# TakiRyo/object-triggered-3D-SLAM

Hardware: AMD Instinct MI355X
Metric: RGB-D frames/sec (640×480, 5mm voxel TSDF) at 1/2/4/8 GPU; Mpoints/s filtered (higher is better)
Workload: dtype f32 tsdf/weight + f64 colour; 1 GPU; configs[1]: 256-frame 640x480 RGB-D TSDF integration, 5 mm voxel, sdf_trunc 0.04, one object scan per GPU (synthetic box-on-floor ring scan), colour precision 64 (Open3D's float64 TSDFVoxel::color_, exact division: bit-exact colours); color_precision=64, width=640, height=480, volume_units=5896, parallelism=objects1

## Files before the change

### object-triggered-3d-slam_amd/_lib.py

```python
from __future__ import annotations

import ctypes as C
import os
import threading

_HERE = os.path.dirname(os.path.abspath(__file__))
LIB_PATH = os.path.join(_HERE, "libotslam_hip.so")
HEADER_PATH = os.path.join(os.path.dirname(_HERE), "include", "otslam.h")

OT_OK = 0
OT_ERR_INVALID_ARGUMENT = 1
OT_ERR_UNSUPPORTED_FORMAT = 2
OT_ERR_CAPACITY = 3
OT_ERR_HIP = 4

OT_COLOR_NONE = 0
OT_COLOR_RGB8 = 1


class ot_intrinsics(C.Structure):
    _fields_ = [("width", C.c_int32), ("height", C.c_int32), ("fx", C.c_double), ("fy", C.c_double),
                ("cx", C.c_double), ("cy", C.c_double)]


# ... 56 lines not shown
    "ot_tsdf_import_units": [_p, _i64, _p, _p, _p, _p, _p],
    "ot_tsdf_import_units_color64": [_p, _i64, _p, _p, _p, _p, _p],
    "ot_tsdf_set_shard": [_p, _i32, _i32],
    "ot_tsdf_set_shard_block": [_p, _i32],
    "ot_tsdf_set_shard_sector": [_p, _i32, _i32, _d, _d],
    "ot_tsdf_batch_stats": [_p, _pi64, _pi64, _pi64],
    "ot_tsdf_border_destinations": [_p, _i64, _p, _p, _p],
    "ot_tsdf_mesh_serial": [_p, _pi64],
    "ot_tsdf_mesh_vertex_normals": [_p, _i64, _p, _i64, _p, _i64, _p, _p],
    "ot_tsdf_export_border": [_p, _i64, _p, _p, _p, _p, _pi64, _p],
    "ot_tsdf_import_border": [_p, _i64, _p, _p, _p, _p, _p],
    "ot_tsdf_fetch_mesh_keys": [_p, _p, _p, _p],
    "ot_tsdf_extract_triangle_mesh": [_p, _pi64, _pi64, _p],
    "ot_tsdf_fetch_triangle_mesh": [_p, _p, _p, _p, _p],
    "ot_tsdf_extract_triangle_mesh_count": [_p, _pi64, _pi64, _p],
    "ot_tsdf_emit_triangle_mesh": [_p, _p, _p, _p, _p],
    "ot_tsdf_extract_triangle_mesh_into": [_p, _p, _p, _p, _i64, _i64, _pi64, _pi64, _p],
    "ot_tsdf_extract_sample_min_z": [_p, _p, _p, _p, _i64, _i64, _p, _p, _i64, C.c_uint64, _d, _p, _p, _pi64, _pi64,
                                     _pi64, _p],
    "ot_tsdf_extract_point_cloud_count": [_p, _pi64, _p],
    "ot_tsdf_emit_point_cloud": [_p, _p, _p, _p, _p],
    "ot_tsdf_extract_voxel_point_cloud_count": [_p, _pi64, _p],
    "ot_tsdf_emit_voxel_point_cloud": [_p, _p, _p, _p],
    "ot_mesh_compute_vertex_normals": [_p, _i64, _p, _i64, _p, _p],
    "ot_mesh_sample_points_uniformly": [_p, _p, _p, _i64, _p, _i64, _i64, C.c_uint64, _p, _p, _p, _p],
    "ot_mesh_sample_points_uniformly_batch": [_p, _i32, _i64, C.c_uint64, _p],
    "ot_mesh_sample_points_min_z": [_p, _i32, _i64, C.c_uint64, _d, _pi64, _p],
    "ot_mesh_sample_points_min_z_async": [_p, _i32, _i64, C.c_uint64, _d, _p],
    "ot_mesh_sample_points_min_z_wait": [_i32, _pi64],
    "ot_mesh_sample_points_uniformly_after": [_p, _i32, _i64, C.c_uint64, _p, _p],
    "ot_mesh_get_surface_area": [_p, _i64, _p, _i64, C.POINTER(C.c_double), _p],
    "ot_mesh_cluster_connected_triangles": [_p, _i64, _p, _i64, _p, _p, _p, _pi64, _p],
    "ot_mesh_flag_degenerate_triangles": [_p, _i64, _i64, _p, _p],
    "ot_mesh_flag_duplicated_triangles": [_p, _i64, _i64, _p, _p],
    "ot_mesh_remove_triangles_by_mask": [_p, _i64, _p, _p, _pi64, _p],
    "ot_mesh_remove_unreferenced_vertices": [_i64, _p, _i64, _p, _pi64, _p],
    "ot_occupancy_to_points": [_p, _i32, _i32, _i32, _d, _d, _d, _p, _pi64, _p],
    "ot_grid_smart_paste": [_p, _p, _i32, _i32, _i32, _i32, _i32, _i32, _i32, _i32, _pi64, _p],
    "ot_voxel_key_diff": [_p, _i64, _p, _i64, _d, _p, _p, _pi64, _p, _pi64, _p],
    "ot_voxel_key_diff_multi": [_p, _p, _p, _p, _i32, _d, _p, _p, _pi64, _p, _pi64, _p],
    "ot_scan_diff": [_p, _p, _i32, _i32, C.c_float, C.c_float, C.c_float, C.c_float, C.c_float, _d, _i32, _p, _d,
                     _p, _p, _p, _p, _p],
    "ot_virtual_scan": [_p, _i32, _i32, C.c_float, C.c_float, C.c_float, _i32, _i32, C.c_float, C.c_float,
                        C.c_float, _p, _p, _p],
    "ot_change_grid_create": [_d, _d, _d, C.POINTER(_p)],
    "ot_change_grid_destroy": [_p],
    "ot_change_grid_update": [_p, _p, _p, _i64, _d],
    "ot_change_grid_publish": [_p, _p, _i64, _pi64],
    "ot_scan_cluster": [_p, _i32, _i32, C.c_float, C.c_float, C.c_float, _p, _p, _p, _p, _p, _p, _p, _p, _p, _p, _p,
                        _p],
    "ot_object_map_filter": [_p, _p, _i32, _p, _i32, C.c_float, C.c_float, C.c_float, _p, _d, _p, _p, _p, _p],
    "ot_cluster_observations": [_p, _i32, _p, _i32, _p, _p, _p, _p, _p],
    "ot_rgbd_filter_create": [_pint, _i32, _d, _d, _d, _i32, _d, C.POINTER(_p)],
    "ot_rgbd_filter_destroy": [_p],
    "ot_rgbd_filter_run": [_p, _i32, _p, _p, _p, _p],
    "ot_rgbd_filter_sizes": [_p, _pi64, _pi64, _pi64, _p, _p, _p],
    "ot_rgbd_filter_outputs": [_p, C.POINTER(_p), C.POINTER(_p), C.POINTER(_p), C.POINTER(_p), C.POINTER(_p),
                               C.POINTER(_p)],
    "ot_rgbd_filter_copy": [_p, _i32, _p, _p, _p, _p, _p, _p, _p],
}
_RESTYPES = {"ot_last_error": C.c_char_p, "ot_version": C.c_char_p, "ot_abi_version": C.c_int32,
             "otx_alloc_count": C.c_longlong}

_lib = None
_lock = threading.Lock()


class OTError(RuntimeError):
    """Raised for any non-OK status; message mirrors Open3D's utility::LogError text."""


TEST_SIGNATURES = {
    "otx_serial_chain_f64": [_p, _i64, _i32, _p, _pi64, _p],
    "otx_chain_walk_trace": [_p, _i64, _i32, _p, _p, _i32, _p],
    "otx_tsdf_stats": [_p, _p],
    "otx_unit_sort_radix": [_i32],
    "otx_sor_netfill": [_i32],
    "otx_integrate_fine": [_i32],
    "otx_integrate_workgroup": [_i32],
    "otx_touch_stage_blocks": [_i32],
    "otx_touch_frames": [_i32],
    "otx_split_frontend": [_i32],
    "otx_slice_pretest": [_i32],
    "otx_defer_integrate": [_i32],
    "otx_integrate_depth": [_i32],
    "otx_mc_emit_fork": [_i32],
    "otx_normals_at": [_i32],
    "otx_sampler_hi_stream": [_i32],
    "otx_sort_pairs_u64_u32": [_p, _p, _p, _p, _i64, _i32, _p],
    "otx_sort_segments_u32_u32": [_p, _p, _p, _p, _p, _i32, _i32, _p],
    "otx_alloc_count": [],
    "otx_registration_last_d2": [_p, _i64, _p],
}


def use_variant(path: str) -> None:
    global LIB_PATH
    path = os.path.abspath(path)
    if os.path.dirname(path) != os.path.join(_HERE, "variants"):
        raise RuntimeError(f"variant libraries live in {os.path.join(_HERE, 'variants')}: {path}")
    if _lib is not None:
        raise RuntimeError("use_variant() after the library was loaded")
    LIB_PATH = path


def load():
    global _lib
    if _lib is not None:
        return _lib
    with _lock:
        if _lib is not None:
            return _lib
        if not os.path.exists(LIB_PATH):
            raise RuntimeError(f"HIP extension missing: {LIB_PATH} (run __graft_entry__.build())")
        lib = C.CDLL(LIB_PATH)
        lib.ot_version.argtypes, lib.ot_version.restype = [], C.c_char_p
        built, src = library_source_hash(lib), source_hash()
        if built != src:
            raise RuntimeError(f"stale HIP library {LIB_PATH}: built from sources {built or '(no hash)'}, "
                               f"sources here are {src} (run __graft_entry__.build())")
        missing = []
        for name, argtypes in {**SIGNATURES, **TEST_SIGNATURES}.items():
            try:
                f = getattr(lib, name)
            except AttributeError:
                missing.append(name)
                continue
            f.argtypes = argtypes
            f.restype = _RESTYPES.get(name, C.c_int32)
        lib._ot_missing = set(missing)
        _lib = lib
    return _lib


def call(name, *args):
    lib = load()
    if name in lib._ot_missing:
        raise RuntimeError(f"{LIB_PATH} does not export {name} (stale build?)")
    st = getattr(lib, name)(*args)
    if st != OT_OK:
        msg = lib.ot_last_error().decode(errors="replace")
        raise OTError(msg or f"{name} failed with status {st}")
    return st


def alloc_count() -> int:
    return int(load().otx_alloc_count())


def intrinsics_struct(intr) -> ot_intrinsics:
    return ot_intrinsics(int(intr.width), int(intr.height), float(intr.fx), float(intr.fy), float(intr.cx),
                         float(intr.cy))


def source_hash() -> str:
    from . import _srchash

    return _srchash.compute()


def library_source_hash(lib) -> str:
    ver = lib.ot_version().decode(errors="replace")
    return ver.rsplit(" src=", 1)[1].strip() if " src=" in ver else ""
```

### object-triggered-3d-slam_amd/csrc/tsdf.h

```cpp
#pragma once

#include <vector>

#include "common.h"

namespace ot {

constexpr int UNIT_RES = 16;
constexpr int UNIT_VOX = UNIT_RES * UNIT_RES * UNIT_RES;
constexpr int UNIT_FIELDS = 5;
constexpr int UNIT_FLOATS = UNIT_FIELDS * UNIT_VOX;
constexpr int UNIT_FLOATS_C64 = 8 * UNIT_VOX;

constexpr int C_UNUSED0 = 0;
constexpr int C_UNITS = 1;
constexpr int C_OVERFLOW = 2;
constexpr int C_HASHERR = 3;
constexpr int C_BATCH_PAIRS = 4;
constexpr int C_ORDER_HEAVY = 6;
constexpr int C_ORDER_LIGHT = 7;
constexpr int C_KMAX = 8;
constexpr int C_KNEG = 11;
constexpr int C_UNITS_DONE = 14;
constexpr int N_COUNTERS = 16;
// ... 83 lines not shown
    }
    return -1;
}

__device__ inline int hash_find(const TsdfDev& d, unsigned long long key) {
    unsigned slot = (unsigned)mix64(key) & (unsigned)d.hash_mask;
    for (int probe = 0; probe <= d.hash_mask; ++probe) {
        const unsigned long long k = d.hkeys[slot];
        if (k == key) return (int)slot;
        if (k == KEY_EMPTY) return -1;
        slot = (slot + 1) & (unsigned)d.hash_mask;
    }
    return -1;
}

__host__ __device__ inline float* unit_base(const TsdfDev& d, int id) { return d.vox + (size_t)id * d.unit_floats; }
template <typename CT>
__device__ inline CT* color_base(const TsdfDev& d, int id) {
    return reinterpret_cast<CT*>(unit_base(d, id) + 2 * UNIT_VOX);
}

constexpr int BORDER_VOX = 721;
__host__ __device__ inline void border_voxel(int b, int& x, int& y, int& z) {
    if (b < 256) {
        x = 0, y = b >> 4, z = b & 15;
        return;
    }
    const int c = b - 256, r = c % 31;
    x = 1 + c / 31;
    if (r < 16) y = 0, z = r;
    else y = r - 15, z = 0;
}

constexpr int MAX_BATCH = 64;
constexpr int OT_MAIL_WORDS = 64;
constexpr int MAIL_SEQ_MC = OT_MAIL_WORDS - 2;
constexpr int MAIL_SEQ_UNITS = 2 * OT_MAIL_WORDS - 1;

struct BatchFrame {
    const uint16_t* depth16;
    const float* depthf;
    const uint8_t* color;
    uint2* dc;
    uint64_t pad;
    double pose[12];
    float E[12];
    float es[3];
    float scale;
    double trunc;
};

struct IntegrateParams {
    const float* depth;
    const uint8_t* color;
    const float* mult;
    int W, H;
    float fx, fy, cx, cy;
    float E[12];
    float es0, es1, es2;
    float vl, half, trunc, trunc_inv, safe_w, safe_h;
    float inv_fx, inv_fy;
    float proj_eps;
    int rcp_hi;
    double unit_len;
    const unsigned* tmax;
    int tmax_tiles;
    int tmax_words;
};

struct BatchTouchParams {
    int W, stride, ws, hs;
    double fx, fy, cx, cy;
    double trunc, unit_len;
    double inv_unit;
    int slot_cap;
    int64_t npx;
    int pc;
    int tiles;
    int stage_blocks;
    int tf;
    int sample_stage;
    unsigned* tmax;
    int H;
};

struct StageMaskParams {
    int W, H, tiles_x, tiles_y, wpr;
    float fx, fy, cx, cy, vl, half;
    double unit_len;
    int nframes;
};

struct UnitWork {
    int id;
    int kx, ky, kz;
    unsigned long long mask;
    unsigned long long pad;
};

enum class BatchMode { Direct, Overlap, Deferred };
struct BatchPlan {
    BatchMode mode = BatchMode::Direct;
    bool split = false;
    bool pretest = false;
    int set = 0;
    int* wcount = nullptr;
    int* wcopy = nullptr;
};

struct BatchCtx {
    BatchPlan plan;
    BatchTouchParams tp;
    IntegrateParams ip0;
    StageMaskParams sq{};
    unsigned* smask = nullptr;
    int n, pc, variant;
};

struct PendingFrame {
    const uint16_t* depth;
    const float* depthf;
    const uint8_t* color;
    ot_intrinsics intr;
    double extrinsic[16];
    double depth_scale, depth_trunc;
};

struct MeshBuffers {
    void* ws = nullptr;
    size_t ws_bytes = 0;
    int64_t ws_units = 0;
    int64_t serial = 0;
    bool valid = false;
    bool internal = false;
    bool emitted = false;
    double* v = nullptr;
    double* c = nullptr;
    int32_t* t = nullptr;
    int4* vk = nullptr;
    int* vown = nullptr;
    int32_t* tk = nullptr;
    int64_t nv = 0, nt = 0;
    int64_t cap_v = 0, cap_t = 0, cap_vk = 0, cap_tk = 0, cap_vown = 0;
};

struct CloudBuffers {
    void* ws = nullptr;
    size_t ws_bytes = 0;
    int64_t units = 0;
    int64_t n_surface = 0, n_voxel = 0;
    bool valid = false;
};

}

struct ot_tsdf {
    int device = 0;
    double voxel_length = 0.0, sdf_trunc = 0.0, unit_length = 0.0;
    int color_type = 1, stride = 4;
    bool color64 = false;
    int64_t max_units = 0;
    int64_t hash_cap = 0;
    ot::TsdfDev dev{};
    int frame_id = 0;
    bool imported = false;
    float* mult = nullptr;
    ot_intrinsics mult_intr{};
    bool mult_valid = false;
    int batch_max = ot::MAX_BATCH;
    std::vector<ot::PendingFrame> pending;
    ot::BatchFrame* hbframes = nullptr;
    unsigned* hmail = nullptr;
    int hb_next = 0;
    unsigned units_seq = 0;
    int early_frame = -1;
    unsigned mc_seq = 0;
    int batch_pc = ot::C_BATCH_PAIRS;
    struct BatchSet {
        ot::BatchFrame* bframes = nullptr;
        uint2* bdc = nullptr;
        int64_t cap = 0;
        unsigned* tmax = nullptr;
        int64_t tmax_cap = 0;
        void* work = nullptr;
        hipEvent_t ev_units = nullptr;
        hipEvent_t ev_done = nullptr;
    } bset[2];
    int overlap_mode = -1;
    unsigned* tmask = nullptr;
    int64_t tmask_words = 0;
    int tmask_w = 0, tmask_h = 0;
    int split_mode = -1;
    bool dfr_on = false;
    hipStream_t dfr_stream = nullptr;
    hipEvent_t ev_dfr = nullptr;
    ot::BatchCtx dfr;
    int64_t stat_batches = 0, stat_unit_batches = 0, stat_fresh = 0, stat_prev_units = 0;
    int64_t last_batch_slots = -1;
    int bset_next = 0;
    int last_set = -1;
    hipStream_t istream = nullptr;
    int* wcount = nullptr;
    unsigned* sorted_ids = nullptr;
    int64_t sorted_units = -1;
    int sorted_frame = -1;
    ot::MeshBuffers mesh;
    ot::CloudBuffers cloud;
    hipStream_t side = nullptr;
    hipEvent_t ev_fork = nullptr, ev_join = nullptr;
    hipEvent_t ev_normals = nullptr;
    bool normals_pending = false;
    hipEvent_t ev_made = nullptr;
    bool profiling = false;
    std::vector<std::pair<hipEvent_t, hipEvent_t>> prof_events;
    double prof_ms = 0.0;
    int64_t prof_launches = 0;
    std::vector<std::pair<hipEvent_t, hipEvent_t>> prof_fe_events;
    double prof_fe_ms = 0.0;
    int64_t prof_fe_batches = 0;
};

namespace ot {
struct TsdfHooks {
    int int_fine = -1;
    int fine_units = -1;
    int int_depth = -1;
    int int_wg = -1;
    int stage_blocks = -1;
    int touch_tf = -1;
    int split = -1;
    int defer = -1;
    int pretest = -1;
    bool unit_sort_radix = false;
};
extern TsdfHooks g_tsdf_hooks;

ot_status reserve_units(ot_tsdf* vol, int64_t extra, hipStream_t stream);
ot_status export_list(ot_tsdf* vol, hipStream_t stream, const unsigned** ids, int64_t* n);
ot_status tsdf_sorted_units(ot_tsdf* vol, hipStream_t stream, int64_t* n_units);
struct MailSrc {
    const unsigned* p[ot::OT_MAIL_WORDS];
    int n;
};
ot_status mail_words(ot_tsdf* vol, const MailSrc& s, hipStream_t stream);
ot_status mail_wait(const unsigned* word, unsigned seq, hipStream_t stream);
ot_status tsdf_flush(ot_tsdf* vol, hipStream_t stream, bool join = true);
ot_status wait_normals(ot_tsdf* vol, hipStream_t stream);
ot_status sample_min_z_enqueue(const ot_mesh_sample_job* jobs, int32_t n_jobs, int64_t n_points, uint64_t seed,
                               double z_min, hipStream_t stream, hipStream_t* hs, hipEvent_t mark = nullptr,
                               int mark_at = 0);
ot_status sample_min_z_wait(hipStream_t hs, int32_t n_jobs, int64_t* n_kept_host);
}
```

### object-triggered-3d-slam_amd/csrc/tsdf.hip

```cpp
#include <algorithm>
#include <cmath>
#include <cstring>
#include <type_traits>
#include <utility>

#include "slice_pretest.h"
#include "tsdf.h"

namespace ot {

typedef unsigned u32x2 __attribute__((ext_vector_type(2)));
typedef unsigned u32x4 __attribute__((ext_vector_type(4)));

__device__ inline __amdgpu_buffer_rsrc_t make_rsrc(const void* base, int bytes) {
    return __builtin_amdgcn_make_buffer_rsrc(const_cast<void*>(base), (short)0, bytes, 0x00020000);
}

__device__ inline double ld_f64(__amdgpu_buffer_rsrc_t r, int i) {
    const u32x2 v = __builtin_amdgcn_raw_buffer_load_b64(r, i * 8, 0, 0);
    return __hiloint2double((int)v.y, (int)v.x);
}
__device__ inline void st_f64(__amdgpu_buffer_rsrc_t r, int i, double x) {
    u32x2 v;
    v.x = (unsigned)__double2loint(x);
    v.y = (unsigned)__double2hiint(x);
    __builtin_amdgcn_raw_buffer_store_b64(v, r, i * 8, 0, 0);
}

__device__ inline float prep_depth(const BatchFrame& fr, uint32_t raw16) {
    float dv = (float)raw16;
    dv = dv / fr.scale;
    if ((double)dv >= fr.trunc) dv = 0.0f;
    return dv;
}

__device__ inline void store_quad(uint2* dc, float d0, float d1, float d2, float d3, uint32_t w0, uint32_t w1,
                                  uint32_t w2) {
    const uint32_t p0 = w0 & 0xFFFFFFu;
    const uint32_t p1 = (w0 >> 24) | ((w1 & 0xFFFFu) << 8);
    const uint32_t p2 = (w1 >> 16) | ((w2 & 0xFFu) << 16);
    const uint32_t p3 = w2 >> 8;
    uint4* q = reinterpret_cast<uint4*>(dc);
    q[0] = make_uint4(__float_as_uint(d0), p0, __float_as_uint(d1), p1);
    q[1] = make_uint4(__float_as_uint(d2), p2, __float_as_uint(d3), p3);
}

__device__ inline void prep_quad(const BatchFrame& fr, int64_t i0, int64_t npx) {
    const bool aligned = ((reinterpret_cast<uintptr_t>(fr.depth16) & 7) == 0) &&
                         ((reinterpret_cast<uintptr_t>(fr.depthf) & 15) == 0) &&
                         ((reinterpret_cast<uintptr_t>(fr.color) & 3) == 0);
    if (aligned && i0 + 4 <= npx && (npx & 3) == 0) {
        float d[4];
        if (fr.depth16) {
            const uint2 raw = *reinterpret_cast<const uint2*>(fr.depth16 + i0);
            d[0] = prep_depth(fr, raw.x & 0xFFFFu);
            d[1] = prep_depth(fr, raw.x >> 16);
            d[2] = prep_depth(fr, raw.y & 0xFFFFu);
            d[3] = prep_depth(fr, raw.y >> 16);
        } else {
            const float4 v = *reinterpret_cast<const float4*>(fr.depthf + i0);
            d[0] = v.x, d[1] = v.y, d[2] = v.z, d[3] = v.w;
        }
        uint32_t w0 = 0u, w1 = 0u, w2 = 0u;
        if (fr.color) {
            const uint32_t* c = reinterpret_cast<const uint32_t*>(fr.color + i0 * 3);
            w0 = c[0], w1 = c[1], w2 = c[2];
        }
        store_quad(fr.dc + i0, d[0], d[1], d[2], d[3], w0, w1, w2);
    } else {
        for (int64_t i = i0; i < npx && i < i0 + 4; ++i) {
            const float dv = fr.depth16 ? prep_depth(fr, fr.depth16[i]) : fr.depthf[i];
            uint32_t cw = 0u;
            if (fr.color) {
                const uint8_t* c = fr.color + i * 3;
                cw = (uint32_t)c[0] | ((uint32_t)c[1] << 8) | ((uint32_t)c[2] << 16);
            }
            fr.dc[i] = make_uint2(__float_as_uint(dv), cw);
        }
    }
}

constexpr int PREP_K = 2;
__device__ inline void prep_range(const BatchFrame& fr, int64_t q, int64_t q1, int64_t npx) {
    const bool fast = fr.depth16 && fr.color && (npx & 3) == 0 &&
                      ((reinterpret_cast<uintptr_t>(fr.depth16) & 7) == 0) &&
                      ((reinterpret_cast<uintptr_t>(fr.color) & 3) == 0);
    if (fast) {
        for (; q + 256 * (PREP_K - 1) < q1; q += 256 * PREP_K) {
            uint2 raw[PREP_K];
            uint32_t w[PREP_K][3];
#pragma unroll
            for (int k = 0; k < PREP_K; ++k) {
                const int64_t i0 = (q + 256 * k) * 4;
                raw[k] = *reinterpret_cast<const uint2*>(fr.depth16 + i0);
                const uint32_t* c = reinterpret_cast<const uint32_t*>(fr.color + i0 * 3);
                w[k][0] = c[0], w[k][1] = c[1], w[k][2] = c[2];
            }
#pragma unroll
            for (int k = 0; k < PREP_K; ++k) {
                const int64_t i0 = (q + 256 * k) * 4;
                const float d0 = prep_depth(fr, raw[k].x & 0xFFFFu), d1 = prep_depth(fr, raw[k].x >> 16);
                const float d2 = prep_depth(fr, raw[k].y & 0xFFFFu), d3 = prep_depth(fr, raw[k].y >> 16);
                store_quad(fr.dc + i0, d0, d1, d2, d3, w[k][0], w[k][1], w[k][2]);
            }
        }
    }
    for (; q < q1; q += 256) prep_quad(fr, q * 4, npx);
}

static_assert(sizeof(BatchFrame) % 16 == 0, "BatchFrame is copied in 16-B words");
constexpr int COPY_FRAMES_LANES = 1024;
static_assert(sizeof(BatchFrame) / 16 * MAX_BATCH <= COPY_FRAMES_LANES, "one word per lane");
__global__ __launch_bounds__(COPY_FRAMES_LANES) void k_copy_frames(const uint4* __restrict__ src,
                                                                   uint4* __restrict__ dst, int n16) {
    const int i = threadIdx.x;
    if (i < n16) dst[i] = src[i];
}
// ... 12 lines not shown
        return;
    }
    const unsigned long long key = pack_key(x, y, z);
    if (!unit_owned(d, key)) return;
    const int slot = hash_insert(d, key);
    if (slot < 0) {
        atomicOr(&d.counters[C_HASHERR], 1);
        return;
    }
    const unsigned long long bit = 1ull << f;
    if (d.fmask[slot] & bit) return;
    const unsigned long long old = atomicOr(&d.fmask[slot], bit);
    if (old == 0ull) {
        const int pos = atomicAdd(&d.counters[pc], 1);
        if (pos < slot_cap) d.bslots[pos] = slot;
        else atomicOr(&d.counters[C_HASHERR], 1);
    }
}

constexpr int TT = 16;
constexpr int TF = 2;
constexpr int LTAB = 1024;

__device__ inline bool lds_merge(unsigned long long* keys, unsigned long long* masks, unsigned short* used, int* nused,
                                 unsigned long long key, unsigned long long bit) {
    unsigned h = (unsigned)mix64(key) & (LTAB - 1);
    for (int probe = 0; probe < 64; ++probe) {
        unsigned long long k = keys[h];
        if (k == KEY_EMPTY) {
            const unsigned long long old = atomicCAS(&keys[h], KEY_EMPTY, key);
            if (old == KEY_EMPTY) used[atomicAdd(nused, 1)] = (unsigned short)h;
            k = (old == KEY_EMPTY) ? key : old;
        }
        if (k == key) {
            atomicOr(&masks[h], bit);
            return true;
        }
        h = (h + 1) & (LTAB - 1);
    }
    return false;
}

__device__ inline unsigned group8_max(unsigned v) {
    v = max(v, (unsigned)__shfl_xor((int)v, 1));
    v = max(v, (unsigned)__shfl_xor((int)v, 2));
    return max(v, (unsigned)__shfl_xor((int)v, 4));
}
__device__ __noinline__ void tile_max_range(const BatchFrame& fr, unsigned* __restrict__ map, int W, int H, int i0,
                                            int step) {
    const int tmx = pre_tiles(W), total = tmx * pre_tiles(H) * PRE_TILE;
    const bool rows16 = fr.depth16 && (W & 7) == 0 && (reinterpret_cast<uintptr_t>(fr.depth16) & 15) == 0;
    for (int i = i0; i < total; i += step) {
        const int t = i >> 3, y = (t / tmx) * PRE_TILE + (i & 7), x0 = (t % tmx) * PRE_TILE;
        const int cols = min(PRE_TILE, W - x0);
        const bool inside = y < H;
        unsigned key = 0u;
        bool done = false;
        if (rows16) {
            unsigned m = 0u;
            if (inside) {
                const uint4 v = *reinterpret_cast<const uint4*>(fr.depth16 + (int64_t)y * W + x0);
                const unsigned w4[4] = {v.x, v.y, v.z, v.w};
#pragma unroll
                for (int k = 0; k < 4; ++k) m = max(m, max(w4[k] & 0xFFFFu, w4[k] >> 16));
            }
            m = group8_max(m);
            const float d = prep_depth(fr, m);
            done = m == 0u || d > 0.0f;
            key = pre_depth_key(d);
        }
        if (!done) {
            key = 0u;
            if (inside)
                for (int c = 0; c < cols; ++c) {
                    const int64_t px = (int64_t)y * W + x0 + c;
                    key = max(key, pre_depth_key(fr.depth16 ? prep_depth(fr, fr.depth16[px]) : fr.depthf[px]));
                }
            key = group8_max(key);
        }
        if ((i & 7) == 0) map[t] = key;
    }
}

__device__ inline void stage_share(const BatchFrame* __restrict__ frames, const BatchTouchParams& p, int nframes,
                                   int grp, int part, int parts) {
    const int64_t quads = (p.npx + 3) >> 2;
    const int64_t per = (quads + parts - 1) / parts;
    const int64_t q0 = (int64_t)part * per, q1 = q0 + per < quads ? q0 + per : quads;
    for (int f = grp * p.tf; f < grp * p.tf + p.tf && f < nframes; ++f) {
        prep_range(frames[f], q0 + threadIdx.x, q1, p.npx);
        if (p.tmax)
            tile_max_range(frames[f], p.tmax + (size_t)f * (pre_tiles(p.W) * pre_tiles(p.H)), p.W, p.H,
                           part * 256 + (int)threadIdx.x, parts * 256);
    }
}

struct TouchLds {
    unsigned long long keys[LTAB];
    unsigned long long masks[LTAB];
    unsigned short used[LTAB];
    int nused;
};
template <bool REPLAY, bool STAGE = !REPLAY>
__device__ __forceinline__ void touch_body(const BatchFrame* __restrict__ frames, const BatchTouchParams& p,
                                           const TsdfDev& d, int nframes, TouchLds& L, int tile, int grp) {
    unsigned long long* s_keys = L.keys;
    unsigned long long* s_masks = L.masks;
    unsigned short* s_used = L.used;
    int& s_nused = L.nused;
    const int tid = threadIdx.x;
    if constexpr (STAGE) {
        if (p.stage_blocks > 0 && tile >= p.tiles) {
            stage_share(frames, p, nframes, grp, tile - p.tiles, p.stage_blocks);
            return;
        }
    }
    for (int e = tid; e < LTAB; e += 256) {
        s_keys[e] = KEY_EMPTY;
        s_masks[e] = 0ull;
    }
    if (tid == 0) s_nused = 0;
    if constexpr (STAGE) {
        if (p.stage_blocks == 0) stage_share(frames, p, nframes, grp, tile, p.tiles);
    }
    __syncthreads();
    const int tiles_x = (p.ws + TT - 1) / TT;
    const int sx = (tile % tiles_x) * TT + (tid & (TT - 1));
    const int sy = (tile / tiles_x) * TT + (tid / TT);
    const int f0 = grp * p.tf;
    if (sx < p.ws && sy < p.hs) {
        const int r = sy * p.stride, c = sx * p.stride;
        for (int f = f0; f < f0 + p.tf && f < nframes; ++f) {
            const BatchFrame& fr = frames[f];
            const int64_t pix = (int64_t)r * p.W + c;
            const float df = REPLAY           ? __uint_as_float(fr.dc[pix].x)
                             : fr.depth16 ? prep_depth(fr, fr.depth16[pix])
                                          : fr.depthf[pix];
            if constexpr (!REPLAY) {
                if (p.sample_stage) {
                    uint32_t cw = 0u;
                    if (fr.color) {
                        const uint8_t* c = fr.color + pix * 3;
                        cw = (uint32_t)c[0] | ((uint32_t)c[1] << 8) | ((uint32_t)c[2] << 16);
                    }
                    fr.dc[pix] = make_uint2(__float_as_uint(df), cw);
                }
            }
            if (!(df > 0.0f)) continue;
            const double z = (double)df;
            const double x = ((double)c - p.cx) * z / p.fx;
            const double y = ((double)r - p.cy) * z / p.fy;
            double q[3];
#pragma unroll
            for (int k = 0; k < 3; ++k) {
                const double a = fr.pose[k * 4 + 0] * x;
                const double b = fr.pose[k * 4 + 1] * y;
                const double cc = fr.pose[k * 4 + 2] * z;
                q[k] = ((a + b) + cc) + fr.pose[k * 4 + 3];
            }
            int lo[3], hi[3];
#pragma unroll
            for (int k = 0; k < 3; ++k) {
                lo[k] = floor_div(q[k] - p.trunc, p.unit_len, p.inv_unit);
                hi[k] = floor_div(q[k] + p.trunc, p.unit_len, p.inv_unit);
            }
            const unsigned long long bit = 1ull << f;
            for (int ux = lo[0]; ux <= hi[0]; ++ux)
                for (int uy = lo[1]; uy <= hi[1]; ++uy)
                    for (int uz = lo[2]; uz <= hi[2]; ++uz) {
                        if (!key_in_range(ux, uy, uz)) {
                            atomicOr(&d.counters[C_HASHERR], 2);
                            continue;
// ... 1025 lines not shown
    note_alloc();
    const size_t rec = sizeof(float) * (size_t)d.unit_floats;
    if (n_used > 0) {
        OT_HIP_TRY(hipMemcpyAsync(nd.vox, d.vox, rec * n_used, hipMemcpyDeviceToDevice, stream));
        OT_HIP_TRY(hipMemcpyAsync(nd.unit_keys, d.unit_keys, sizeof(int) * 3 * n_used, hipMemcpyDeviceToDevice, stream));
        OT_HIP_TRY(hipMemcpyAsync(nsorted, vol->sorted_ids, sizeof(unsigned) * n_used, hipMemcpyDeviceToDevice, stream));
    }
    OT_HIP_TRY(hipMemsetAsync(nd.hkeys, 0xFF, sizeof(unsigned long long) * cap, stream));
    OT_HIP_TRY(hipMemsetAsync(nd.hvals, 0xFF, sizeof(int) * cap, stream));
    OT_HIP_TRY(hipMemsetAsync(nd.fmask, 0, sizeof(unsigned long long) * cap, stream));
    nd.hash_mask = (int)(cap - 1);
    nd.max_units = (int)nmax;
    if (n_used > 0) hipLaunchKernelGGL(k_rehash, dim3((unsigned)((n_used + 255) / 256)), dim3(256), 0, stream, nd, n_used);
    OT_LAUNCH_CHECK();
    OT_HIP_TRY(hipStreamSynchronize(stream));
    for (void* p : {(void*)d.vox, (void*)d.unit_keys, (void*)vol->sorted_ids, (void*)d.hkeys, (void*)d.hvals,
                    (void*)d.fmask, (void*)d.bslots, d.work, vol->bset[1].work})
        if (p) (void)hipFree(p);
    d = nd;
    vol->bset[1].work = work1;
    vol->sorted_ids = nsorted;
    vol->max_units = nmax;
    vol->hash_cap = cap;
    return OT_OK;
}


static ot_status plan_batch(ot_tsdf* vol, const ot_intrinsics& in, int pc, BatchPlan& p) {
    p.split = split_on(vol) && tmask_fits(in.width, in.height);
    const int pre = g_tsdf_hooks.pretest;
    p.pretest = !p.split && (pre > 0 || (pre < 0 && vol->dev.shard_world <= 1)) &&
                (int64_t)pre_tiles(in.width) * pre_tiles(in.height) * MAX_BATCH + PRE_SLACK < (int64_t)PRE_NONE;
    p.mode = defer_on(vol, p.split) ? BatchMode::Deferred : overlap_on(vol) ? BatchMode::Overlap : BatchMode::Direct;
    p.wcount = vol->dev.counters + pc;
    if (p.mode != BatchMode::Direct) {
        ot_status st = ensure_overlap(vol);
        if (st != OT_OK) return st;
        p.set = vol->bset_next;
        vol->bset_next ^= 1;
        p.wcount = p.wcopy = vol->wcount + p.set;
    }
    return OT_OK;
}

static void fill_batch_frames(const ot_tsdf* vol, const PendingFrame* frames, int n, uint2* bdc, int64_t npx, float vl,
                              BatchFrame* host) {
    for (int k = 0; k < n; ++k) {
        const PendingFrame& f = frames[k];
        BatchFrame& b = host[k];
        b.depth16 = f.depth;
        b.depthf = f.depth ? nullptr : f.depthf;
        b.color = (vol->color_type == OT_COLOR_RGB8) ? f.color : nullptr;
        b.dc = bdc + npx * k;
        b.pad = 0;
        double pose[16];
        inverse4(f.extrinsic, pose);
        for (int i = 0; i < 12; ++i) b.pose[i] = pose[i];
        float E[12];
        for (int i = 0; i < 12; ++i) b.E[i] = E[i] = (float)f.extrinsic[i];
        for (int i = 0; i < 3; ++i) b.es[i] = E[i * 4 + 2] * vl;
        b.scale = (float)f.depth_scale;
        b.trunc = f.depth_trunc;
    }
}

static BatchTouchParams make_touch_params(const ot_tsdf* vol, const ot_intrinsics& in, int pc, bool split) {
    BatchTouchParams tp;
    tp.npx = (int64_t)in.width * in.height;
    tp.pc = pc;
    tp.W = in.width, tp.stride = vol->stride;
    tp.ws = (in.width + vol->stride - 1) / vol->stride;
    tp.hs = (in.height + vol->stride - 1) / vol->stride;
    tp.fx = in.fx, tp.fy = in.fy, tp.cx = in.cx, tp.cy = in.cy;
    tp.trunc = vol->sdf_trunc;
    tp.unit_len = vol->unit_length, tp.inv_unit = 1.0 / vol->unit_length;
    tp.slot_cap = (int)vol->hash_cap;
    tp.tiles = ((tp.ws + TT - 1) / TT) * ((tp.hs + TT - 1) / TT);
    tp.stage_blocks = g_tsdf_hooks.stage_blocks < 0 ? 2 * tp.tiles : g_tsdf_hooks.stage_blocks;
    tp.tf = g_tsdf_hooks.touch_tf > 0 ? g_tsdf_hooks.touch_tf : TF;
    tp.sample_stage = split ? 1 : 0;
    if (split) tp.stage_blocks = -1;
    tp.tmax = nullptr;
    tp.H = in.height;
    return tp;
}

static StageMaskParams make_stage_params(const ot_tsdf* vol, const ot_intrinsics& in, const IntegrateParams& ip, int n) {
    StageMaskParams q;
    q.W = in.width, q.H = in.height;
    q.tiles_x = (in.width + STX - 1) / STX;
    q.tiles_y = (in.height + STY - 1) / STY;
    q.wpr = (q.tiles_x + 31) / 32;
    q.fx = ip.fx, q.fy = ip.fy, q.cx = ip.cx, q.cy = ip.cy;
    q.vl = ip.vl, q.half = ip.half;
    q.unit_len = vol->unit_length;
    q.nframes = n;
    return q;
}

struct ProfPair {
    hipEvent_t e0 = nullptr, e1 = nullptr;
};
static ot_status prof_open(const ot_tsdf* vol, ProfPair& p, hipStream_t stream) {
    if (!vol->profiling) return OT_OK;
    OT_HIP_TRY(hipEventCreate(&p.e0));
    OT_HIP_TRY(hipEventCreate(&p.e1));
    OT_HIP_TRY(hipEventRecord(p.e0, stream));
    return OT_OK;
}
static ot_status prof_close(const ProfPair& p, hipStream_t stream, decltype(ot_tsdf::prof_events)& list) {
    if (!p.e0) return OT_OK;
    OT_HIP_TRY(hipEventRecord(p.e1, stream));
    list.emplace_back(p.e0, p.e1);
    return OT_OK;
}

static void launch_front_end(ot_tsdf* vol, const BatchCtx& bc, bool replay, bool touch, hipStream_t stream) {
    const BatchPlan& plan = bc.plan;
    const BatchFrame* bf = vol->bset[plan.set].bframes;
    UnitWork* work = (UnitWork*)set_work(vol, plan.set);
    BatchTouchParams tp = bc.tp;
    tp.slot_cap = (int)vol->hash_cap;
    if (touch) {
        const auto touch_k = replay ? k_batch_touch<true> : plan.split ? k_batch_touch_split : k_batch_touch<false>;
        const unsigned tiles = (unsigned)tp.tiles + (replay ? 0u : (unsigned)std::max(0, tp.stage_blocks));
        hipLaunchKernelGGL(touch_k, dim3(tiles, (unsigned)((bc.n + tp.tf - 1) / tp.tf)), dim3(256), 0, stream, bf, tp,
                           vol->dev, bc.n);
    }
    const bool missing_only = replay && plan.mode != BatchMode::Deferred;
    int* wcopy = missing_only ? nullptr : plan.wcopy;
    const auto units_k = missing_only ? k_batch_units<true> : k_batch_units<false>;
    hipLaunchKernelGGL(units_k, dim3(256), dim3(256), 0, stream, vol->dev, work, bc.pc, vol->hmail + OT_MAIL_WORDS, wcopy,
                       ++vol->units_seq);
    if (plan.split)
        launch_stage(bf, bc.sq, (const UnitWork*)work, (const int*)(wcopy ? wcopy : vol->dev.counters + bc.pc), bc.smask,
                     stream);
}

static ot_status launch_integrate(ot_tsdf* vol, const BatchCtx& bc, int variant, const int* wcount, hipStream_t stream) {
    const BatchFrame* bf = vol->bset[bc.plan.set].bframes;
    const UnitWork* uw = (const UnitWork*)set_work(vol, bc.plan.set);
    void* args[] = {(void*)&bf, (void*)&bc.ip0, (void*)&vol->dev, (void*)&uw, (void*)&wcount};
    const IntForm f = integrate_form(variant, bc.ip0.rcp_hi);
    OT_HIP_TRY(hipLaunchKernel(f.fn, dim3(f.grid), dim3(64 * f.wg), args, f.lds, stream));
    OT_LAUNCH_CHECK();
    return OT_OK;
}

static ot_status follow_deferred(ot_tsdf* vol, hipStream_t stream) {
    if (stream == vol->dfr_stream) return OT_OK;
    if (!vol->ev_dfr) OT_HIP_TRY(hipEventCreateWithFlags(&vol->ev_dfr, hipEventDisableTiming));
    OT_HIP_TRY(hipEventRecord(vol->ev_dfr, vol->dfr_stream));
    OT_HIP_TRY(hipStreamWaitEvent(stream, vol->ev_dfr, 0));
    vol->dfr_stream = stream;
    return OT_OK;
}

static ot_status launch_deferred(ot_tsdf* vol, hipStream_t stream, const BatchCtx* next) {
    if (!vol->dfr_on) return OT_OK;
    ot_status st = follow_deferred(vol, stream);
    if (st != OT_OK) return st;
    vol->dfr_on = false;
    const BatchCtx& D = vol->dfr;
    const int variant = slice_form(D.variant & 3, vol->last_batch_slots, true);
    ProfPair timed;
    if ((st = prof_open(vol, timed, stream)) != OT_OK) return st;
// ... 31 lines not shown
            ++vol->stat_batches;
            vol->stat_unit_batches += c[bc.pc];
        }
        const bool short_of_room = c[C_OVERFLOW] != 0 || (c[C_HASHERR] & 1) != 0;
        if (!short_of_room) {
            if (vol->stat_prev_units >= 0) vol->stat_fresh += c[C_UNITS] - vol->stat_prev_units;
            vol->stat_prev_units = c[C_UNITS];
            if ((int64_t)c[C_UNITS] * 4 > vol->max_units * 3)
                return grow_pool(vol, (int64_t)c[C_UNITS] * 2, c[C_UNITS], stream);
            return OT_OK;
        }
        if (round >= 8) return fail(OT_ERR_CAPACITY, "[ScalableTSDFVolume] unit pool: growth did not converge");
        const int used = (int)std::min<int64_t>(c[C_UNITS], vol->max_units);
        const int64_t need = std::max<int64_t>((int64_t)c[C_UNITS], vol->max_units) + 1;
        ot_status st = grow_pool(vol, need, used, stream);
        if (st != OT_OK) return st;
        int h[N_COUNTERS];
        OT_HIP_TRY(hipMemcpy(h, vol->dev.counters, sizeof(h), hipMemcpyDeviceToHost));
        h[C_UNITS] = used;
        h[C_OVERFLOW] = 0;
        h[C_HASHERR] &= ~1;
        h[bc.pc] = 0;
        OT_HIP_TRY(hipMemcpy(vol->dev.counters, h, sizeof(h), hipMemcpyHostToDevice));
        launch_front_end(vol, bc, true, true, stream);
        if (bc.plan.mode == BatchMode::Deferred) {
            OT_LAUNCH_CHECK();
            continue;
        }
        st = launch_integrate(vol, bc, bc.variant, vol->dev.counters + bc.pc, stream);
        if (st != OT_OK) return st;
        vol->last_set = -1;
        vol->sorted_frame = -1;
    }
}

static ot_status integrate_batch(ot_tsdf* vol, const PendingFrame* frames, int n, hipStream_t stream) {
    const ot_intrinsics& in = frames[0].intr;
    ot_status st = wait_normals(vol, stream);
    if (st != OT_OK || (st = ensure_mult(vol, &in, stream)) != OT_OK) return st;
    BatchCtx bc;
    bc.pc = vol->batch_pc;
    bc.n = n;
    if ((st = plan_batch(vol, in, bc.pc, bc.plan)) != OT_OK) return st;
    const BatchPlan& plan = bc.plan;
    if (vol->dfr_on) {
        if ((st = follow_deferred(vol, stream)) != OT_OK) return st;
        if (plan.mode != BatchMode::Deferred && (st = launch_deferred(vol, stream, nullptr)) != OT_OK) return st;
    }
    auto& bs = vol->bset[plan.set];
    if (plan.mode == BatchMode::Overlap) OT_HIP_TRY(hipStreamWaitEvent(stream, bs.ev_done, 0));
    const int64_t npx = (int64_t)in.width * in.height;
    if (bs.cap < npx * n) {
        if (bs.bdc) {
            OT_HIP_TRY(hipStreamSynchronize(stream));
            if (vol->istream) OT_HIP_TRY(hipStreamSynchronize(vol->istream));
            OT_HIP_TRY(hipFree(bs.bdc));
            bs.bdc = nullptr;
        }
        const int64_t cap = npx * std::max(n, std::min(vol->batch_max, MAX_BATCH));
        OT_HIP_TRY(hipMalloc(&bs.bdc, sizeof(uint2) * cap));
        bs.cap = cap;
    }
    BatchFrame* host = vol->hbframes + vol->hb_next * MAX_BATCH;
    vol->hb_next ^= 1;
    bc.ip0 = make_integrate_params(vol, nullptr, nullptr, vol->mult, &in, frames[0].extrinsic);
    fill_batch_frames(vol, frames, n, bs.bdc, npx, bc.ip0.vl, host);
    hipLaunchKernelGGL(k_copy_frames, dim3(1), dim3(COPY_FRAMES_LANES), 0, stream, (const uint4*)host,
                       (uint4*)bs.bframes, (int)(sizeof(BatchFrame) / 16) * n);
    bc.tp = make_touch_params(vol, in, bc.pc, plan.split);
    if (plan.pretest) {
        const int64_t tiles = (int64_t)pre_tiles(in.width) * pre_tiles(in.height);
        if (bs.tmax_cap < tiles * n) {
            if (bs.tmax) {
                OT_HIP_TRY(hipStreamSynchronize(stream));
                if (vol->istream) OT_HIP_TRY(hipStreamSynchronize(vol->istream));
                OT_HIP_TRY(hipFree(bs.tmax));
                bs.tmax = nullptr, bs.tmax_cap = 0;
            }
            const int64_t cap = tiles * std::max(n, std::min(vol->batch_max, MAX_BATCH));
            OT_HIP_TRY(hipMalloc(&bs.tmax, sizeof(unsigned) * (cap + PRE_SLACK)));
            bs.tmax_cap = cap;
        }
        bc.tp.tmax = bs.tmax;
        bc.ip0.tmax = bs.tmax;
        bc.ip0.tmax_tiles = (int)tiles;
        bc.ip0.tmax_words = (int)(tiles * n);
    }
    if (plan.split) {
        if ((st = ensure_tmask(vol, in.width, in.height, stream)) != OT_OK) return st;
        bc.sq = make_stage_params(vol, in, bc.ip0, n);
        bc.smask = vol->tmask;
    }
    const bool fast = !vol->imported && (int64_t)vol->frame_id + n < RCP_N;
    bc.variant = (vol->color64 ? 2 : 0) + (fast ? 1 : 0);
    bc.ip0.rcp_hi = (int)std::min<int64_t>((int64_t)vol->frame_id + n, RCP_N);
    if (plan.mode != BatchMode::Deferred) bc.variant = slice_form(bc.variant, direct_estimate(vol), false);

    ProfPair fe;
    if ((st = prof_open(vol, fe, stream)) != OT_OK) return st;
    const bool fused = plan.mode == BatchMode::Deferred && vol->dfr_on;
    if (fused && (st = launch_deferred(vol, stream, &bc)) != OT_OK) return st;
    launch_front_end(vol, bc, false, !fused, stream);
    if (plan.mode == BatchMode::Deferred) {
        if ((st = prof_close(fe, stream, vol->prof_fe_events)) != OT_OK) return st;
        vol->dfr = bc;
        vol->dfr_on = true, vol->dfr_stream = stream;
    } else {
        hipStream_t is = stream;
        if (plan.mode == BatchMode::Overlap) {
            OT_HIP_TRY(hipEventRecord(bs.ev_units, stream));
            OT_HIP_TRY(hipStreamWaitEvent(vol->istream, bs.ev_units, 0));
            is = vol->istream;
        }
        if ((st = prof_close(fe, stream, vol->prof_fe_events)) != OT_OK) return st;
        ProfPair timed;
        if ((st = prof_open(vol, timed, is)) != OT_OK) return st;
        if ((st = launch_integrate(vol, bc, bc.variant, plan.wcount, is)) != OT_OK) return st;
        if ((st = prof_close(timed, is, vol->prof_events)) != OT_OK) return st;
        if (plan.mode == BatchMode::Overlap) {
            OT_HIP_TRY(hipEventRecord(bs.ev_done, is));
            vol->last_set = plan.set;
        }
    }
    vol->batch_pc ^= 1;
    vol->frame_id += n;
    vol->sorted_frame = -1;
    vol->early_frame = vol->frame_id;
    return settle_batch(vol, bc, stream);
}

ot_status reserve_units(ot_tsdf* vol, int64_t extra, hipStream_t stream) {
    int nu = 0;
    OT_HIP_TRY(hipMemcpyAsync(&nu, vol->dev.counters + C_UNITS, sizeof(int), hipMemcpyDeviceToHost, stream));
    OT_HIP_TRY(hipStreamSynchronize(stream));
    const int used = (int)std::min<int64_t>(nu, vol->max_units);
    if (used + extra <= vol->max_units) return OT_OK;
    return grow_pool(vol, used + extra, used, stream);
}

ot_status wait_normals(ot_tsdf* vol, hipStream_t stream) {
    if (!vol->normals_pending) return OT_OK;
    const hipError_t q = hipEventQuery(vol->ev_normals);
    if (q == hipSuccess) {
        vol->normals_pending = false;
        return OT_OK;
    }
    if (q != hipErrorNotReady) OT_HIP_TRY(q);
    OT_HIP_TRY(hipStreamWaitEvent(stream, vol->ev_normals, 0));
    return OT_OK;
}

ot_status tsdf_flush(ot_tsdf* vol, hipStream_t stream, bool join) {
    size_t i = 0;
    std::vector<PendingFrame> frames;
    frames.swap(vol->pending);
    if (!frames.empty()) vol->mesh.valid = vol->cloud.valid = false;
    while (i < frames.size()) {
        size_t n = 1;
        const int cap = std::min(vol->batch_max, MAX_BATCH);
        while (i + n < frames.size() && (int)n < cap &&
               std::memcmp(&frames[i + n].intr, &frames[i].intr, sizeof(ot_intrinsics)) == 0)
            ++n;
        ot_status st = integrate_batch(vol, frames.data() + i, (int)n, stream);
        if (st != OT_OK) return st;
        i += n;
    }
    if (!join) return OT_OK;
    ot_status st = launch_deferred(vol, stream, nullptr);
    if (st != OT_OK) return st;
    return join_integrate(vol, stream);
}

}

using namespace ot;

extern "C" {

ot_status ot_tsdf_integrate(ot_tsdf* vol, const float* depth, const uint8_t* color, const ot_intrinsics* in,
                            const double extrinsic[16], void* stream) {
    ot_status st = check_frame(vol, depth, color, in, extrinsic);
    if (st != OT_OK) return st;
    PendingFrame f;
    f.depth = nullptr;
    f.depthf = depth;
    f.color = color;
    f.intr = *in;
    std::memcpy(f.extrinsic, extrinsic, sizeof(double) * 16);
    f.depth_scale = 1.0;
    f.depth_trunc = 0.0;
    vol->pending.push_back(f);
    if ((int)vol->pending.size() >= std::min(vol->batch_max, MAX_BATCH)) return tsdf_flush(vol, S(stream), false);
    return OT_OK;
}

ot_status ot_tsdf_integrate_u16(ot_tsdf* vol, const uint16_t* depth, const uint8_t* color, const ot_intrinsics* in,
                                const double extrinsic[16], double depth_scale, double depth_trunc, void* stream) {
    ot_status st = check_frame(vol, depth, color, in, extrinsic);
    if (st != OT_OK) return st;
    PendingFrame f;
    f.depth = depth;
    f.depthf = nullptr;
    f.color = color;
    f.intr = *in;
    std::memcpy(f.extrinsic, extrinsic, sizeof(double) * 16);
    f.depth_scale = depth_scale;
    f.depth_trunc = depth_trunc;
// ... 26 lines not shown
```

### object-triggered-3d-slam_amd/csrc/tsdf_volume.hip

```cpp
#include <algorithm>
#include <chrono>
#include <cmath>
#include <cstring>
#include <sched.h>
#include <thread>

#include "tsdf.h"

namespace ot {

TsdfHooks g_tsdf_hooks;

static void reset_host_state(ot_tsdf* v) {
    v->batch_pc = C_BATCH_PAIRS;
    v->frame_id = 0;
    v->imported = false;
    v->early_frame = -1;
    v->last_batch_slots = -1;
    v->stat_batches = v->stat_unit_batches = v->stat_fresh = v->stat_prev_units = 0;
    v->sorted_frame = -1;
    v->sorted_units = -1;
    v->mesh.nv = v->mesh.nt = 0;
    v->mesh.valid = false;
    v->cloud.valid = false;
}

__global__ void k_mail_words(MailSrc s, unsigned* __restrict__ out) {
    const int i = threadIdx.x;
    if (i < s.n) out[i] = *s.p[i];
}

ot_status mail_words(ot_tsdf* vol, const MailSrc& s, hipStream_t stream) {
    if (s.n > MAIL_SEQ_MC) return fail(OT_ERR_INVALID_ARGUMENT, "mailbox overflow");
    hipLaunchKernelGGL(k_mail_words, dim3(1), dim3(64), 0, stream, s, vol->hmail);
    OT_LAUNCH_CHECK();
    OT_HIP_TRY(hipStreamSynchronize(stream));
    return OT_OK;
}

ot_status mail_wait(const unsigned* word, unsigned seq, hipStream_t stream) {
    using clk = std::chrono::steady_clock;
    const clk::time_point t0 = clk::now();
    const clk::time_point t_yield = t0 + std::chrono::microseconds(50);
    const clk::time_point t_sleep = t0 + std::chrono::milliseconds(2);
    clk::time_point next = t0 + std::chrono::milliseconds(20);
    for (unsigned it = 1;; ++it) {
        if (__atomic_load_n(word, __ATOMIC_ACQUIRE) == seq) return OT_OK;
        const bool spin = (it & 63u) != 0;
        if (spin && it < (1u << 20)) {
            __builtin_ia32_pause();
            continue;
        }
        const clk::time_point now = clk::now();
        if (now < t_yield) {
            __builtin_ia32_pause();
            continue;
        }
        it = 1u << 20;
        if (now >= next) {
            next = now + std::chrono::milliseconds(1);
            const hipError_t q = hipStreamQuery(stream);
            if (q == hipSuccess) {
                if (__atomic_load_n(word, __ATOMIC_ACQUIRE) == seq) return OT_OK;
                return fail(OT_ERR_HIP, "mailbox: the stream drained without the kernel's mail");
            }
            if (q != hipErrorNotReady) OT_HIP_TRY(q);
        }
        if (now < t_sleep) sched_yield();
        else std::this_thread::sleep_for(std::chrono::microseconds(20));
    }
}

__global__ __launch_bounds__(256) void k_tsdf_clear(TsdfDev d, int64_t cap) {
    for (int64_t i = (int64_t)blockIdx.x * 256 + threadIdx.x; i < cap; i += (int64_t)gridDim.x * 256) {
        d.hkeys[i] = ~0ull;
        d.hvals[i] = -1;
        d.fmask[i] = 0ull;
    }
    if (blockIdx.x == 0) {
        if (threadIdx.x < N_COUNTERS) d.counters[threadIdx.x] = 0;
        for (int i = threadIdx.x; i < N_STATS; i += 256) d.stats[i] = 0ull;
    }
}

}

using namespace ot;

extern "C" {
// ... 269 lines not shown
    for (int i = 0; i < S_DROP_LINES; ++i) {
        out4[S_PRETEST_DROPPED] += s[S_DROP_BASE + i * S_DROP_STRIDE];
        out4[S_UPDATES] += s[S_UPD_BASE + i * S_DROP_STRIDE];
    }
    return OT_OK;
}

ot_status otx_integrate_fine(int32_t mode) {
    g_tsdf_hooks.int_fine = mode < 0 ? -1 : (mode == 1 ? 1 : 0);
    g_tsdf_hooks.fine_units = mode >= 2 ? mode : -1;
    return OT_OK;
}

ot_status otx_integrate_workgroup(int32_t waves) {
    if (waves != -1 && waves != 1 && waves != 2 && waves != 4)
        return fail(OT_ERR_INVALID_ARGUMENT, "otx_integrate_workgroup: -1, 1, 2 or 4 waves");
    g_tsdf_hooks.int_wg = waves;
    return OT_OK;
}

ot_status otx_touch_stage_blocks(int32_t blocks) {
    if (blocks > 4096) return fail(OT_ERR_INVALID_ARGUMENT, "otx_touch_stage_blocks: at most 4096");
    g_tsdf_hooks.stage_blocks = blocks < 0 ? -1 : blocks;
    return OT_OK;
}

ot_status otx_touch_frames(int32_t tf) {
    if (tf < 1 || tf > MAX_BATCH) return fail(OT_ERR_INVALID_ARGUMENT, "otx_touch_frames: 1..64");
    g_tsdf_hooks.touch_tf = tf;
    return OT_OK;
}

ot_status otx_unit_sort_radix(int32_t on) {
    g_tsdf_hooks.unit_sort_radix = on != 0;
    return OT_OK;
}

ot_status ot_tsdf_set_shard(ot_tsdf* vol, int32_t rank, int32_t world) {
    if (!vol || world < 1 || rank < 0 || rank >= world)
        return fail(OT_ERR_INVALID_ARGUMENT, "[ScalableTSDFVolume] shard needs 0 <= rank < world");
    int nu = 0;
    OT_HIP_TRY(hipMemcpy(&nu, vol->dev.counters + C_UNITS, sizeof(int), hipMemcpyDeviceToHost));
    if (nu != 0 || !vol->pending.empty())
        return fail(OT_ERR_INVALID_ARGUMENT, "[ScalableTSDFVolume] set the shard before the first integrate");
    vol->dev.shard_rank = rank;
    vol->dev.shard_world = world;
    vol->dev.shard_mode = SHARD_BLOCKS;
    vol->dev.shard_shift = world <= 4 ? 2 : 1;
    return OT_OK;
}

ot_status ot_tsdf_set_shard_sector(ot_tsdf* vol, int32_t rank, int32_t world, double cx, double cy) {
    if (!vol || world < 1 || rank < 0 || rank >= world || !std::isfinite(cx) || !std::isfinite(cy))
        return fail(OT_ERR_INVALID_ARGUMENT, "[ScalableTSDFVolume] shard needs 0 <= rank < world and a finite centre");
    const double hx = std::nearbyint(2.0 * cx / vol->unit_length), hy = std::nearbyint(2.0 * cy / vol->unit_length);
    if (std::fabs(hx) > (double)(1 << 22) || std::fabs(hy) > (double)(1 << 22))
        return fail(OT_ERR_INVALID_ARGUMENT, "[ScalableTSDFVolume] sector centre out of the unit key range");
    ot_status st = ot_tsdf_set_shard(vol, rank, world);
    if (st != OT_OK) return st;
    vol->dev.shard_mode = SHARD_SECTORS;
    vol->dev.shard_cx2 = (int)hx;
    vol->dev.shard_cy2 = (int)hy;
    return OT_OK;
}

ot_status otx_integrate_depth(int32_t kt) {
    if (kt != -1 && (kt < 1 || kt > 3)) return fail(OT_ERR_INVALID_ARGUMENT, "integrate pipeline depth must be -1 or 1..3");
    g_tsdf_hooks.int_depth = kt;
    return OT_OK;
}

ot_status otx_defer_integrate(int32_t mode) {
    if (mode < -1 || mode > 1) return fail(OT_ERR_INVALID_ARGUMENT, "deferred integrate mode must be -1, 0 or 1");
    g_tsdf_hooks.defer = mode;
    return OT_OK;
}

ot_status otx_slice_pretest(int32_t mode) {
    if (mode < -1 || mode > 1) return fail(OT_ERR_INVALID_ARGUMENT, "slice pre-test mode must be -1, 0 or 1");
    g_tsdf_hooks.pretest = mode;
    return OT_OK;
}

ot_status otx_split_frontend(int32_t mode) {
    if (mode < -1 || mode > 1) return fail(OT_ERR_INVALID_ARGUMENT, "split front end mode must be -1, 0 or 1");
    g_tsdf_hooks.split = mode;
    return OT_OK;
}

ot_status ot_tsdf_set_shard_block(ot_tsdf* vol, int32_t log2_units) {
    if (!vol || log2_units < 0 || log2_units > 8)
        return fail(OT_ERR_INVALID_ARGUMENT, "[ScalableTSDFVolume] shard block must be 2^0 .. 2^8 units per axis");
    int nu = 0;
    OT_HIP_TRY(hipMemcpy(&nu, vol->dev.counters + C_UNITS, sizeof(int), hipMemcpyDeviceToHost));
    if (nu != 0 || !vol->pending.empty())
        return fail(OT_ERR_INVALID_ARGUMENT, "[ScalableTSDFVolume] set the shard before the first integrate");
    vol->dev.shard_shift = log2_units;
    return OT_OK;
}

}
```

Measured before the change: 94870 frames/s.

## Fuse depth/colour staging and tile-max map into one tile-ordered pass

Adds a one-pass staging path that reads depth and colour per 4x2-pixel quad in tile order, writes the packed depth/colour records, and reduces the per-tile max depth key with wave shuffles in the same loop. This replaces the separate prep_range and tile_max_range passes, which read the frame twice. When the path is active it also resizes the staging block count to the tile count. A test hook and a readback entry point for staged records are added; the path is on by default when alignment conditions hold.

New measurement: 96890 frames/s (median of 6 runs). +2.1%, better.

```diff
diff --git a/object-triggered-3d-slam_amd/_lib.py b/object-triggered-3d-slam_amd/_lib.py
--- a/object-triggered-3d-slam_amd/_lib.py
+++ b/object-triggered-3d-slam_amd/_lib.py
@@ -162,6 +162,8 @@
     "otx_touch_frames": [_i32],
     "otx_split_frontend": [_i32],
     "otx_slice_pretest": [_i32],
+    "otx_stage_onepass": [_i32],
+    "otx_tsdf_staged": [_p, _i32, _p, _p],
     "otx_defer_integrate": [_i32],
     "otx_integrate_depth": [_i32],
     "otx_mc_emit_fork": [_i32],
diff --git a/object-triggered-3d-slam_amd/csrc/tsdf.h b/object-triggered-3d-slam_amd/csrc/tsdf.h
--- a/object-triggered-3d-slam_amd/csrc/tsdf.h
+++ b/object-triggered-3d-slam_amd/csrc/tsdf.h
@@ -189,6 +189,7 @@
     int sample_stage;
     unsigned* tmax;
     int H;
+    int onepass;
 };
 
 struct StageMaskParams {
@@ -305,6 +306,8 @@
     int64_t stat_batches = 0, stat_unit_batches = 0, stat_fresh = 0, stat_prev_units = 0;
     int64_t last_batch_slots = -1;
     int bset_next = 0;
+    int staged_set = -1, staged_n = 0, staged_w = 0, staged_h = 0;
+    bool staged_map = false;
     int last_set = -1;
     hipStream_t istream = nullptr;
     int* wcount = nullptr;
@@ -338,6 +341,7 @@
     int split = -1;
     int defer = -1;
     int pretest = -1;
+    int onepass = -1;
     bool unit_sort_radix = false;
 };
 extern TsdfHooks g_tsdf_hooks;
diff --git a/object-triggered-3d-slam_amd/csrc/tsdf.hip b/object-triggered-3d-slam_amd/csrc/tsdf.hip
--- a/object-triggered-3d-slam_amd/csrc/tsdf.hip
+++ b/object-triggered-3d-slam_amd/csrc/tsdf.hip
@@ -27,12 +27,13 @@
     __builtin_amdgcn_raw_buffer_store_b64(v, r, i * 8, 0, 0);
 }
 
-__device__ inline float prep_depth(const BatchFrame& fr, uint32_t raw16) {
+__device__ inline float prep_depth(float scale, double trunc, uint32_t raw16) {
     float dv = (float)raw16;
-    dv = dv / fr.scale;
-    if ((double)dv >= fr.trunc) dv = 0.0f;
+    dv = dv / scale;
+    if ((double)dv >= trunc) dv = 0.0f;
     return dv;
 }
+__device__ inline float prep_depth(const BatchFrame& fr, uint32_t raw16) { return prep_depth(fr.scale, fr.trunc, raw16); }
 
 __device__ inline void store_quad(uint2* dc, float d0, float d1, float d2, float d3, uint32_t w0, uint32_t w1,
                                   uint32_t w2) {
@@ -211,12 +212,72 @@
     }
 }
 
+typedef const uint32_t __attribute__((address_space(1))) * gc_u32;
+typedef u32x4 __attribute__((address_space(1))) * g_u32x4;
+typedef unsigned __attribute__((address_space(1))) * g_u32;
+__device__ inline bool stage_onepass(const BatchFrame& fr, int W) {
+    return fr.depth16 && (reinterpret_cast<uintptr_t>(fr.depth16) & 15) == 0 && (W & 7) == 0 &&
+           (reinterpret_cast<uintptr_t>(fr.color) & 3) == 0;
+}
+typedef const u32x2 __attribute__((address_space(1))) * gc_u32x2;
+__device__ __noinline__ void stage_tile_quads(const BatchFrame& fr, unsigned* map, int W, int H, int i0, int step) {
+    const int tmx = W >> 3, ntiles = tmx * pre_tiles(H), total = ((ntiles + 7) >> 3) * 64;
+    const BatchFrame __attribute__((address_space(1)))* g = (const BatchFrame __attribute__((address_space(1)))*)&fr;
+    const uint16_t* depth = g->depth16;
+    const uint8_t* color = g->color;
+    uint2* dc = g->dc;
+    const float scale = g->scale;
+    const double trunc = g->trunc;
+    for (int i = i0; i < total; i += step) {
+        const int c = i & 15, t = (i >> 6) * 8 + (c >> 1), tc = min(t, ntiles - 1);
+        const int ty = tc / tmx, y = ty * PRE_TILE + ((i >> 4) & 3), x = (tc - ty * tmx) * PRE_TILE + (c & 1) * 4;
+        const int rows = t < ntiles ? (y + 4 < H ? 2 : y < H ? 1 : 0) : 0;
+        int64_t px[2];
+        u32x2 raw[2];
+        uint32_t w[2][3] = {{0u, 0u, 0u}, {0u, 0u, 0u}};
+#pragma unroll
+        for (int k = 0; k < 2; ++k) {
+            px[k] = (int64_t)min(y + 4 * k, H - 1) * W + x;
+            raw[k] = *(gc_u32x2)(depth + px[k]);
+        }
+        if (color) {
+#pragma unroll
+            for (int k = 0; k < 2; ++k) {
+                gc_u32 cw = (gc_u32)(color + px[k] * 3);
+                w[k][0] = cw[0], w[k][1] = cw[1], w[k][2] = cw[2];
+            }
+        }
+        unsigned key = 0u;
+#pragma unroll
+        for (int k = 0; k < 2; ++k)
+            if (k < rows) {
+                const float d0 = prep_depth(scale, trunc, raw[k].x & 0xFFFFu), d1 = prep_depth(scale, trunc, raw[k].x >> 16);
+                const float d2 = prep_depth(scale, trunc, raw[k].y & 0xFFFFu), d3 = prep_depth(scale, trunc, raw[k].y >> 16);
+                const uint32_t w0 = w[k][0], w1 = w[k][1], w2 = w[k][2];
+                g_u32x4 out = (g_u32x4)(dc + px[k]);
+                out[0] = u32x4{__float_as_uint(d0), w0 & 0xFFFFFFu, __float_as_uint(d1), (w0 >> 24) | ((w1 & 0xFFFFu) << 8)};
+                out[1] = u32x4{__float_as_uint(d2), (w1 >> 16) | ((w2 & 0xFFu) << 16), __float_as_uint(d3), w2 >> 8};
+                key = max(max(key, max(pre_depth_key(d0), pre_depth_key(d1))),
+                          max(pre_depth_key(d2), pre_depth_key(d3)));
+            }
+        key = max(key, (unsigned)__shfl_xor((int)key, 1));
+        key = max(key, (unsigned)__shfl_xor((int)key, 16));
+        key = max(key, (unsigned)__shfl_xor((int)key, 32));
+        if ((i & 0x31) == 0 && t < ntiles) *(g_u32)(map + t) = key;
+    }
+}
+
 __device__ inline void stage_share(const BatchFrame* __restrict__ frames, const BatchTouchParams& p, int nframes,
                                    int grp, int part, int parts) {
     const int64_t quads = (p.npx + 3) >> 2;
     const int64_t per = (quads + parts - 1) / parts;
     const int64_t q0 = (int64_t)part * per, q1 = q0 + per < quads ? q0 + per : quads;
     for (int f = grp * p.tf; f < grp * p.tf + p.tf && f < nframes; ++f) {
+        if (p.tmax && p.onepass && stage_onepass(frames[f], p.W)) {
+            unsigned* map = p.tmax + (size_t)f * (pre_tiles(p.W) * pre_tiles(p.H));
+            stage_tile_quads(frames[f], map, p.W, p.H, part * 256 + (int)threadIdx.x, parts * 256);
+            continue;
+        }
         prep_range(frames[f], q0 + threadIdx.x, q1, p.npx);
         if (p.tmax)
             tile_max_range(frames[f], p.tmax + (size_t)f * (pre_tiles(p.W) * pre_tiles(p.H)), p.W, p.H,
@@ -1408,6 +1469,7 @@
     if (split) tp.stage_blocks = -1;
     tp.tmax = nullptr;
     tp.H = in.height;
+    tp.onepass = g_tsdf_hooks.onepass != 0;
     return tp;
 }
 
@@ -1605,6 +1667,8 @@
             bs.tmax_cap = cap;
         }
         bc.tp.tmax = bs.tmax;
+        if (bc.tp.onepass && g_tsdf_hooks.stage_blocks < 0 && bc.tp.stage_blocks > 0 && in.width % PRE_TILE == 0)
+            bc.tp.stage_blocks = (int)((tiles + 31) / 32);
         bc.ip0.tmax = bs.tmax;
         bc.ip0.tmax_tiles = (int)tiles;
         bc.ip0.tmax_words = (int)(tiles * n);
@@ -1646,6 +1710,8 @@
         }
     }
     vol->batch_pc ^= 1;
+    vol->staged_set = plan.set, vol->staged_n = n, vol->staged_w = in.width, vol->staged_h = in.height;
+    vol->staged_map = bc.tp.tmax != nullptr;
     vol->frame_id += n;
     vol->sorted_frame = -1;
     vol->early_frame = vol->frame_id;
diff --git a/object-triggered-3d-slam_amd/csrc/tsdf_volume.hip b/object-triggered-3d-slam_amd/csrc/tsdf_volume.hip
--- a/object-triggered-3d-slam_amd/csrc/tsdf_volume.hip
+++ b/object-triggered-3d-slam_amd/csrc/tsdf_volume.hip
@@ -5,6 +5,7 @@
 #include <sched.h>
 #include <thread>
 
+#include "slice_pretest.h"
 #include "tsdf.h"
 
 namespace ot {
@@ -440,6 +441,30 @@
     return OT_OK;
 }
 
+ot_status otx_stage_onepass(int32_t mode) {
+    if (mode < -1 || mode > 0) return fail(OT_ERR_INVALID_ARGUMENT, "one-pass staging mode must be -1 or 0");
+    g_tsdf_hooks.onepass = mode;
+    return OT_OK;
+}
+
+ot_status otx_tsdf_staged(ot_tsdf* vol, int32_t frame, uint64_t* records_out, uint32_t* map_out) {
+    if (!vol || !records_out) return fail(OT_ERR_INVALID_ARGUMENT, "invalid arguments");
+    ot_status st = tsdf_flush(vol, nullptr);
+    if (st != OT_OK) return st;
+    if (vol->staged_set < 0 || frame < 0 || frame >= vol->staged_n)
+        return fail(OT_ERR_INVALID_ARGUMENT, "otx_tsdf_staged: no such frame in the last batch");
+    if (map_out && !vol->staged_map) return fail(OT_ERR_INVALID_ARGUMENT, "otx_tsdf_staged: the last batch built no map");
+    OT_HIP_TRY(hipDeviceSynchronize());
+    const auto& bs = vol->bset[vol->staged_set];
+    const int64_t npx = (int64_t)vol->staged_w * vol->staged_h;
+    OT_HIP_TRY(hipMemcpy(records_out, bs.bdc + npx * frame, sizeof(uint2) * npx, hipMemcpyDeviceToHost));
+    if (map_out) {
+        const int64_t tiles = (int64_t)pre_tiles(vol->staged_w) * pre_tiles(vol->staged_h);
+        OT_HIP_TRY(hipMemcpy(map_out, bs.tmax + tiles * frame, sizeof(unsigned) * tiles, hipMemcpyDeviceToHost));
+    }
+    return OT_OK;
+}
+
 ot_status otx_split_frontend(int32_t mode) {
     if (mode < -1 || mode > 1) return fail(OT_ERR_INVALID_ARGUMENT, "split front end mode must be -1, 0 or 1");
     g_tsdf_hooks.split = mode;
```
